# dobraczka/kiez

Hardware: AMD Instinct MI355X
Metric: source queries/sec (fit+kneighbors) + recall@k vs reference, 1/2/4/8 GPU (higher is better)
Workload: dtype f16

## Files before the change

kiez_amd/csrc/kz_knn_device.h:

```cpp
#pragma once
#include "kz_common.h"
#include "kz_plan.h"

typedef float f32x16 __attribute__((ext_vector_type(16)));
typedef float f32x4v __attribute__((ext_vector_type(4)));
__device__ __forceinline__ void kz_glds16(const float* gsrc, float* lds_wave_base) {
    __builtin_amdgcn_global_load_lds((const __attribute__((address_space(1))) void*)gsrc,
                                     (__attribute__((address_space(3))) void*)lds_wave_base, 16, 0, 0);
}
__device__ __forceinline__ void kz_glds16_s(const void* sbase_uniform, unsigned lane_byte_off, float* lds_wave_base) {
    const unsigned lds = (unsigned)(uintptr_t)(__attribute__((address_space(3))) void*)lds_wave_base;
    asm volatile("s_mov_b32 m0, %0\n\ts_nop 0\n\tglobal_load_lds_dwordx4 %1, %2"
                 :
                 : "s"(lds), "v"(lane_byte_off), "s"(sbase_uniform)
                 : "memory", "m0");
}
__device__ __forceinline__ void kz_glds4_s(const void* sbase_uniform, unsigned lane_byte_off, float* lds_wave_base) {
    const unsigned lds = (unsigned)(uintptr_t)(__attribute__((address_space(3))) void*)lds_wave_base;
    asm volatile("s_mov_b32 m0, %0\n\ts_nop 0\n\tglobal_load_lds_dword %1, %2"
                 :
                 : "s"(lds), "v"(lane_byte_off), "s"(sbase_uniform)
                 : "memory", "m0");
}
typedef float f32x4e __attribute__((ext_vector_type(4)));
typedef int i32x2e __attribute__((ext_vector_type(2)));
__device__ __forceinline__ float4 kz_nt_load4(const float4* p) {
    const f32x4v v = __builtin_nontemporal_load(reinterpret_cast<const f32x4v*>(p));
    return make_float4(v.x, v.y, v.z, v.w);
}


__host__ __device__ __forceinline__ int kz_list_region(int64_t list_row, const KzListLayout& L) {
    const int qt = (int)(list_row / KZ_TILE);
    int r = 0;
    while (r + 1 < L.n_regions && qt >= L.qt_end[r]) ++r;
    return r;
}
constexpr int KZ_LSTRIDE = 64;
__host__ __device__ __forceinline__ int64_t kz_list_wave_base(int64_t list_row, const KzListLayout& L, int KP, int piece) {
    const int r = kz_list_region(list_row, L);
    const int64_t row0 = r > 0 ? (int64_t)L.qt_end[r - 1] * KZ_TILE : 0;
    const int64_t wb = (list_row - row0) >> 5;
    return L.base[r] + ((wb * L.pieces[r] + piece) * (int64_t)KP) * KZ_LSTRIDE;
}

__host__ __device__ __forceinline__ int64_t kz_list_contig_off(int64_t list_row, const KzListLayout& L, int KP, int piece) {
    const int r = kz_list_region(list_row, L);
    const int64_t row0 = r > 0 ? (int64_t)L.qt_end[r - 1] * KZ_TILE : 0;
    return L.base[r] + ((list_row - row0) * L.pieces[r] + piece) * (int64_t)KP;
}

struct KnnCandParams {
    const float* qpack;
    const float* ypack;
    const float* ybias;
    const int4* work;
    int qt0;
    int n_ytiles;
    int n_qtiles;
    KzListLayout lay;
    int kg;
    float* out_key;
    int* out_idx;
    const float* theta;
    const float* qnbias;
    void* log_keys;
    void* log_meta;
    unsigned long long* log_cnt;
    long long log_cap;
    const float* qfloor;
};

constexpr int KZ_CAND_LDS_BASE = 16384 + 1024;
constexpr int KZ_LOG_CAP = 16;
constexpr int KZ_CAND_LDS = KZ_CAND_LDS_BASE + KZ_LOG_CAP * 256 * 8;

#ifndef KZ_SCAN_CHUNK
#define KZ_SCAN_CHUNK 16
#endif

template <int KP, int LSTRIDE, int CHUNK = KZ_SCAN_CHUNK>
__device__ __forceinline__ void kz_list_replace_min(float* lk, int* li, float v, int idx, float& tau, int& minpos) {
    lk[minpos * LSTRIDE] = v;
    li[minpos * LSTRIDE] = idx;
    float mn = INFINITY;
    int mp = 0;
#pragma unroll
    for (int c0 = 0; c0 < KP; c0 += CHUNK) {
        float kk[CHUNK];
#pragma unroll
        for (int e = 0; e < CHUNK; ++e) kk[e] = lk[(c0 + e) * LSTRIDE];
        __builtin_amdgcn_sched_barrier(0);
#pragma unroll
        for (int e = 0; e < CHUNK; ++e) {
            if (kk[e] < mn) {
                mn = kk[e];
                mp = c0 + e;
            }
        }
    }
    tau = mn;
    minpos = mp;
}


// ... 256 lines not shown
```

kiez_amd/csrc/kz_knn_epi3.h:

```cpp
#pragma once

typedef __attribute__((address_space(3))) float kz_lds_f32;
typedef __attribute__((address_space(3))) int kz_lds_i32;

template <int IN_LDS>
struct KzListRef;
template <>
struct KzListRef<1> {
    kz_lds_f32* k;
    int i_off;
    static constexpr int KSTRIDE = 128, ISTRIDE = 128;
    __device__ __forceinline__ kz_lds_f32* kp() const { return k; }
    __device__ __forceinline__ kz_lds_i32* ip() const { return (kz_lds_i32*)(k + i_off); }
};
template <>
struct KzListRef<0> {
    float* kb;
    int* ib;
    unsigned off;
    static constexpr int KSTRIDE = 1, ISTRIDE = 1;
    __device__ __forceinline__ float* kp() const { return kb + off; }
    __device__ __forceinline__ int* ip() const { return ib + off; }
};
template <>
struct KzListRef<2> {
    kz_lds_f32* k;
    int* ib;
    unsigned off_u, stride;
    static constexpr int KSTRIDE = 128, ISTRIDE = 1;
    __device__ __forceinline__ kz_lds_f32* kp() const { return k; }
    __device__ __forceinline__ int* ip() const {
        unsigned l;
        asm volatile("v_mbcnt_lo_u32_b32 %0, -1, 0\n\tv_mbcnt_hi_u32_b32 %0, -1, %0" : "=v"(l));
        return ib + off_u + (l & 31u) * stride;
    }
};

template <int IN_LDS>
struct KzCandState3 {
    KzListRef<IN_LDS> list;
    float tau;
    int head;
};

struct KzWavePool {
    __attribute__((address_space(3))) f32x4e* keys;
    __attribute__((address_space(3))) i32x2e* meta;
    int cnt;
    int tiles_done, next_merge;
};

struct KzDualRef {
    int qrow0;
};
constexpr int KZ_COL_FLAG = (int)0x80000000;

__device__ __forceinline__ void kz_flush_col3(const KzWavePool& pool, const KzDualRef& du) {
    const int lane = threadIdx.x & 63;
    int n_col = 0;
    for (int e0 = 0; e0 < pool.cnt; e0 += 64) {
        const int e = e0 + lane;
        const bool col = e < pool.cnt && pool.meta[e].x < 0;
        n_col += (int)__popcll(__builtin_amdgcn_ballot_w64(col));
    }
    if (n_col == 0) return;
    typedef __attribute__((address_space(4))) const volatile unsigned long long kz_karg_u64;
    const __attribute__((address_space(4))) char* ka = (const __attribute__((address_space(4))) char*)__builtin_amdgcn_kernarg_segment_ptr();
    f32x4e* log_keys = (f32x4e*)*(kz_karg_u64*)(ka + offsetof(KnnCandParams, log_keys));
    i32x2e* log_meta = (i32x2e*)*(kz_karg_u64*)(ka + offsetof(KnnCandParams, log_meta));
    unsigned long long* log_cnt = (unsigned long long*)*(kz_karg_u64*)(ka + offsetof(KnnCandParams, log_cnt));
    const long long log_cap = (long long)*(kz_karg_u64*)(ka + offsetof(KnnCandParams, log_cap));
    unsigned long long base = 0;
    if (lane == 0) base = __hip_atomic_fetch_add(log_cnt, (unsigned long long)n_col, __ATOMIC_RELAXED, __HIP_MEMORY_SCOPE_AGENT);
    base = ((unsigned long long)__builtin_amdgcn_readfirstlane((int)(base >> 32)) << 32) | (unsigned)__builtin_amdgcn_readfirstlane((int)base);
    for (int e0 = 0; e0 < pool.cnt; e0 += 64) {
        const int e = e0 + lane;
        i32x2e mt;
        mt.x = 0;
        if (e < pool.cnt) mt = pool.meta[e];
        const bool col = mt.x < 0;
        const unsigned long long mask = __builtin_amdgcn_ballot_w64(col);
        if (col) {
            const unsigned long long pos = base + __builtin_amdgcn_mbcnt_hi((unsigned)(mask >> 32), __builtin_amdgcn_mbcnt_lo((unsigned)mask, 0u));
            if ((long long)pos < log_cap) {
                i32x2e mo;
                mo.x = mt.x & 0x7fffffff;
                mo.y = du.qrow0 + (mt.x & 31);
                __builtin_nontemporal_store(pool.keys[e], log_keys + pos);
                __builtin_nontemporal_store(mo, log_meta + pos);
            }
        }
        base += __popcll(mask);
    }
}

template <int KP>
struct KzBlockMin3 {
    static constexpr int NB = KP >= 64 ? 8 : 4;
    static constexpr int BS = KP / NB;
    float bm[NB];
    __device__ __forceinline__ void init(const float v) {
#pragma unroll
        for (int i = 0; i < NB; ++i) bm[i] = v;
    }
};

template <int KP, int IN_LDS>
__device__ __forceinline__ void kz_list_insert3(const KzListRef<IN_LDS>& L, KzBlockMin3<KP>& bs, float v, int idx, float& tau) {
    constexpr int NB = KzBlockMin3<KP>::NB, BS = KzBlockMin3<KP>::BS, S = KzListRef<IN_LDS>::KSTRIDE, SI = KzListRef<IN_LDS>::ISTRIDE;
    float m = bs.bm[0];
    int b = 0;
#pragma unroll
    for (int i = 1; i < NB; ++i) {
        if (bs.bm[i] < m) {
            m = bs.bm[i];
            b = i;
        }
    }
    auto* blk = L.kp() + (b * BS) * S;
    float kk[BS];
#pragma unroll
    for (int jj = 0; jj < BS; ++jj) kk[jj] = blk[jj * S];
    int pos = BS - 1;
#pragma unroll
    for (int jj = BS - 2; jj >= 0; --jj) pos = (kk[jj] == m) ? jj : pos;
    blk[pos * S] = v;
    L.ip()[(b * BS + pos) * SI] = idx;
    float nm = INFINITY;
#pragma unroll
    for (int jj = 0; jj < BS; ++jj) nm = fminf(nm, (jj == pos) ? v : kk[jj]);
    float t = INFINITY;
#pragma unroll
    for (int i = 0; i < NB; ++i) {
        bs.bm[i] = (b == i) ? nm : bs.bm[i];
        t = fminf(t, bs.bm[i]);
    }
    tau = t;
}

template <int KP, int IN_LDS>
__device__ __forceinline__ void kz_insert_group3(const KzListRef<IN_LDS>& L, KzBlockMin3<KP>& bs,
                                                 __attribute__((address_space(3))) f32x4e* entry,
                                                 const __attribute__((address_space(3))) i32x2e* meta, const int half, float& tau) {
    auto row_of = [&]() {
        const int code = meta->x;
        return (code >> 4) * KZ_TILE + ((code >> 2) & 3) * 32 + (code & 3) * 8 + 4 * half;
    };
    {
        const f32x4e kv = *entry;
        const float m = fmaxf(fmaxf(kv.x, kv.y), fmaxf(kv.z, kv.w));
        if (!(m > tau)) return;
        const int slot = kv.x == m ? 0 : (kv.y == m ? 1 : (kv.z == m ? 2 : 3));
        reinterpret_cast<__attribute__((address_space(3))) float*>(entry)[slot] = -INFINITY;
// ... 223 lines not shown
```

kiez_amd/csrc/kz_knn_epi4.h:

```cpp
#pragma once
#include "kz_knn_epi3.h"

struct KzCandState4 {
    KzListRef<1> list;
    float tau[2];
    int head[2];
};

struct KzDualRef4 {
    int qrow0;
};
constexpr int KZ_COL_QH = 0x40000000;

__device__ __forceinline__ void kz_flush_col4(const KzWavePool& pool, const KzDualRef4& du) {
    const int lane = threadIdx.x & 63;
    int n_col = 0;
    for (int e0 = 0; e0 < pool.cnt; e0 += 64) {
        const int e = e0 + lane;
        const bool col = e < pool.cnt && pool.meta[e].x < 0;
        n_col += (int)__popcll(__builtin_amdgcn_ballot_w64(col));
    }
    if (n_col == 0) return;
    typedef __attribute__((address_space(4))) const volatile unsigned long long kz_karg_u64;
    const __attribute__((address_space(4))) char* ka = (const __attribute__((address_space(4))) char*)__builtin_amdgcn_kernarg_segment_ptr();
    f32x4e* log_keys = (f32x4e*)*(kz_karg_u64*)(ka + offsetof(KnnCandParams, log_keys));
    i32x2e* log_meta = (i32x2e*)*(kz_karg_u64*)(ka + offsetof(KnnCandParams, log_meta));
    unsigned long long* log_cnt = (unsigned long long*)*(kz_karg_u64*)(ka + offsetof(KnnCandParams, log_cnt));
    const long long log_cap = (long long)*(kz_karg_u64*)(ka + offsetof(KnnCandParams, log_cap));
    unsigned long long base = 0;
    if (lane == 0) base = __hip_atomic_fetch_add(log_cnt, (unsigned long long)n_col, __ATOMIC_RELAXED, __HIP_MEMORY_SCOPE_AGENT);
    base = ((unsigned long long)__builtin_amdgcn_readfirstlane((int)(base >> 32)) << 32) | (unsigned)__builtin_amdgcn_readfirstlane((int)base);
    for (int e0 = 0; e0 < pool.cnt; e0 += 64) {
        const int e = e0 + lane;
        i32x2e mt;
        mt.x = 0;
        if (e < pool.cnt) mt = pool.meta[e];
        const bool col = mt.x < 0;
        const unsigned long long mask = __builtin_amdgcn_ballot_w64(col);
        if (col) {
            const unsigned long long pos = base + __builtin_amdgcn_mbcnt_hi((unsigned)(mask >> 32), __builtin_amdgcn_mbcnt_lo((unsigned)mask, 0u));
            if ((long long)pos < log_cap) {
                i32x2e mo;
                mo.x = mt.x & 0x3fffffff;
                mo.y = du.qrow0 + ((mt.x & KZ_COL_QH) ? 32 : 0) + (mt.x & 31);
                __builtin_nontemporal_store(pool.keys[e], log_keys + pos);
                __builtin_nontemporal_store(mo, log_meta + pos);
            }
        }
        base += __popcll(mask);
    }
}

template <bool DUAL>
__device__ __forceinline__ void kz_merge_pool4(KzCandState4& st, KzWavePool& pool, const KzDualRef4& du) {
    constexpr int KP = 16;
    const int lane = threadIdx.x & 63;
    if constexpr (DUAL) kz_flush_col4(pool, du);
#pragma unroll 1
    for (int qh = 0; qh < 2; ++qh) {
        const int own = qh ? st.head[1] : st.head[0];
        const int other = __shfl_xor(own, 32, 64);
        float tau = qh ? st.tau[1] : st.tau[0];
        if (lane < 32) {
            KzListRef<1> L = st.list;
            L.k += 32 * qh;
            KzBlockMin3<KP> bs;
            constexpr int NB = KzBlockMin3<KP>::NB, BS = KzBlockMin3<KP>::BS, S = KzListRef<1>::KSTRIDE;
#pragma unroll
            for (int b = 0; b < NB; ++b) {
                float m = INFINITY;
#pragma unroll
                for (int jj = 0; jj < BS; ++jj) m = fminf(m, L.kp()[(b * BS + jj) * S]);
                bs.bm[b] = m;
            }
#pragma unroll 1
            for (int half = 0; half < 2; ++half) {
                int e = half ? other : own;
#pragma unroll 1
                while (e >= 0) {
                    auto* entry = pool.keys + e;
                    const auto* meta = pool.meta + e;
                    e = meta->y;
                    kz_insert_group3<KP, 1>(L, bs, entry, meta, half, tau);
                }
            }
        }
        tau = __shfl(tau, lane & 31, 64);
        if (qh) {
            st.tau[1] = tau;
            st.head[1] = -1;
        } else {
            st.tau[0] = tau;
            st.head[0] = -1;
        }
    }
    pool.cnt = 0;
}

#define KZ_EPI4_APPEND(blk, g4, gi, head, ev, mask)                                                                   \
    do {                                                                                                              \
        if (ev) {                                                                                                     \
            const int pos = pool.cnt + (int)__builtin_amdgcn_mbcnt_hi((unsigned)((mask) >> 32),                       \
                                                                      __builtin_amdgcn_mbcnt_lo((unsigned)(mask), 0u)); \
            f32x4e kv;                                                                                                \
            kv.x = (blk)[4 * (g4)];                                                                                   \
            kv.y = (blk)[4 * (g4) + 1];                                                                               \
            kv.z = (blk)[4 * (g4) + 2];                                                                               \
            kv.w = (blk)[4 * (g4) + 3];                                                                               \
            pool.keys[pos] = kv;                                                                                      \
            { i32x2e mv_; mv_.x = tile * 16 + (gi); mv_.y = (head); pool.meta[pos] = mv_; }                           \
// ... 156 lines not shown
```

kiez_amd/csrc/kz_knn_h16.h:

```cpp
#pragma once
#include <type_traits>

#include "kz_knn_epi3.h"

typedef _Float16 kz_f16x8 __attribute__((ext_vector_type(8)));

#ifndef KZ_H_DMA_LATE
#define KZ_H_DMA_LATE 1
#endif
template <int KP, int WPS, int NSR, bool DUAL = false, bool WIDE = false>
struct KzHCfg {
    static constexpr int TPW = WIDE ? WPS : 1;
    static constexpr bool LDS_LIST = KP <= 32;
    static constexpr bool LISTS_FIT = WPS <= 2 || KP == 16;
    static constexpr int LMODE = (LDS_LIST && LISTS_FIT) ? 1 : (((KP == 64 && WPS <= 2) || (KP == 32 && WPS == 3)) ? 2 : 0);
    static constexpr bool IN_LDS = LMODE == 1;
    static constexpr int RING = WIDE ? 8 : (WPS == 1 ? 8 : ((WPS == 3 || KP == 32 || NSR < 4) ? 4 : 8));
    static constexpr int PERIOD = RING / 2;
    static constexpr int CAP = WPS == 3 ? (KP <= 32 ? (DUAL ? 176 : 192) : 256) : (WPS == 2 && LMODE == 2 && RING == 8 ? (DUAL ? 140 : 156) : 256);
    static constexpr int RING_BYTES = RING * 4096;
    static constexpr int BIAS_OFF = RING_BYTES;
    static constexpr int SYNC_OFF = BIAS_OFF + 1024;
    static constexpr int THETA_OFF = SYNC_OFF + 256;
    static constexpr int POOLK_OFF = THETA_OFF + (DUAL ? 768 + 768 * TPW : 0);
// ... 32 lines not shown
#endif
    const int t_begin = wd.y, t_end = wd.z, s = wd.w;
    const int total = (t_end - t_begin) * NSR;
    const int wq = WIDE ? (wave & 3) : wave;
    const int wq_v = WIDE ? ((tid >> 6) & 3) : (tid >> 6);
    const int tb = WIDE ? (wave >> 2) : 0;
    const bool valid = !WIDE || wd.x + tb < p.n_qtiles;
    const int qt = WIDE ? (valid ? wd.x + tb : p.n_qtiles - 1) : wd.x;

    auto out_list_offset = [&]() { return kz_list_contig_off((int64_t)qt * KZ_TILE + 32 * wq_v + j, p.lay, KP, s); };
    KzCandState3<IN_LDS> st;
    if constexpr (IN_LDS == 1) {
        st.list.k = (kz_lds_f32*)(smem + Cfg::LIST_OFF + tb * Cfg::LIST_BLOCK) + 32 * wq_v + j;
        st.list.i_off = KP * 128;
    } else if constexpr (IN_LDS == 2) {
        st.list.k = (kz_lds_f32*)(smem + Cfg::LIST_OFF + tb * Cfg::LIST_BLOCK) + 32 * wq_v + j;
        st.list.ib = p.out_idx;
        {
            const int64_t row0 = (int64_t)qt * KZ_TILE + 32 * wq;
            const int64_t o0 = kz_list_contig_off(row0, p.lay, KP, s);
            st.list.off_u = (unsigned)o0;
            st.list.stride = (unsigned)(kz_list_contig_off(row0 + 1, p.lay, KP, s) - o0);
        }
    } else {
        st.list.kb = p.out_key;
        st.list.ib = p.out_idx;
        st.list.off = (unsigned)out_list_offset();
    }
    KzWavePool pool;
    pool.keys = (__attribute__((address_space(3))) f32x4e*)(smem + Cfg::POOLK_OFF) + wave * CAP;
    pool.meta = (__attribute__((address_space(3))) i32x2e*)(smem + Cfg::POOLM_OFF) + wave * CAP;
    const float fl = p.qfloor ? p.qfloor[(int64_t)(p.qt0 + qt) * KZ_TILE + 32 * wq_v + j] : -INFINITY;
    if (h == 0 && valid) {
#pragma unroll 4
        for (int e = 0; e < KP; ++e) {
            st.list.kp()[e * KzListRef<IN_LDS>::KSTRIDE] = fl;
            st.list.ip()[e * KzListRef<IN_LDS>::ISTRIDE] = -1;
        }
    }
    if (total <= 0) {
        if constexpr (IN_LDS != 0) {
            const int64_t listoff = out_list_offset();
            if (h == 0 && valid)
                for (int e = 0; e < KP; ++e) {
                    p.out_key[listoff + e] = -INFINITY;
                    if constexpr (IN_LDS == 1) p.out_idx[listoff + e] = -1;
                }
        }
        return;
    }
    st.tau = valid ? fl : INFINITY;
    KzBlockMin3<KP> bmin;
    bmin.init(fl);
    st.head = -1;
    pool.cnt = 0;
    pool.tiles_done = 0;
    pool.next_merge = 1;

    const char* dma_src = reinterpret_cast<const char*>(p.ypack) + ((int64_t)t_begin * NSR) * 4096;
    int dma_slot = 0;
    int dma_turn = 0;
    const int lane_off = (WIDE ? (tid & 255) : tid) * 16;
    auto dma_next = [&]() {
        float* dst = ybuf + dma_slot * 1024 + wq * 256;
        if (!WIDE || tb == dma_turn) kz_glds16_s(dma_src, (unsigned)lane_off, dst);
        if constexpr (WIDE) dma_turn = dma_turn + 1 == TPW ? 0 : dma_turn + 1;
        dma_src += 4096;
        dma_slot = (dma_slot + 1) & (R - 1);
    };
#pragma unroll
    for (int i = 0; i < R; ++i) dma_next();
    bbuf[(t_begin & 1) * 128 + (tid & 127)] = p.ybias[(int64_t)t_begin * KZ_TILE + (tid & 127)];
    KzDualRef du;
    if constexpr (DUAL) {
        if (tid < 64) tbuf[tid] = p.theta[(int64_t)t_begin * KZ_TILE + tid];
        du.qrow0 = (p.qt0 + qt) * KZ_TILE + 32 * wq;
        if (h == 0) tbuf[192 + 32 * (tid >> 6) + j] = valid ? p.qnbias[du.qrow0 + j] : INFINITY;
    }
    if (tid < 4) msync[tid] = 0;
    const float* qbase = p.qpack + ((int64_t)(p.qt0 + qt) * NSR) * 1024 + (h * KZ_TILE + 32 * wq_v + j) * 4;
    kz_f16x8 qf[NSR];
#pragma unroll
    for (int u = 0; u < NSR; ++u) qf[u] = *reinterpret_cast<const kz_f16x8*>(qbase + u * 1024);
    asm volatile("s_waitcnt vmcnt(0)" ::: "memory");
    __syncthreads();

    const float* fbase = ybuf + (h * KZ_TILE + j) * 4;
    kz_f16x8 f0[4], f1[4];
    int dma_due = 0;
    auto fetch_frags = [&](kz_f16x8 (&f)[4], const int gi) {
        const float* fb = fbase + (gi & (R - 1)) * 1024;
#pragma unroll
        for (int mt = 0; mt < 4; ++mt) f[mt] = *reinterpret_cast<const kz_f16x8*>(fb + 128 * mt);
    };
    if (CARRY) fetch_frags(f0, 0);
    int g = 0;
    int th_cur = 0;
    f32x16 acc[4];

    auto run_tile = [&](const int tile, auto start_parity) __attribute__((always_inline)) {
        constexpr int P0 = decltype(start_parity)::value;
        {
            int h_now = h;
            if constexpr (WPS == 3) {
                asm volatile("v_mbcnt_lo_u32_b32 %0, -1, 0\n\tv_mbcnt_hi_u32_b32 %0, -1, %0\n\tv_lshrrev_b32 %0, 5, %0" : "=v"(h_now));
            }
            const float* bp = bbuf + (tile & 1) * 128 + 4 * h_now;
#pragma unroll
            for (int mt = 0; mt < 4; ++mt) {
#pragma unroll
                for (int g4 = 0; g4 < 4; ++g4) {
                    const float4 v = *reinterpret_cast<const float4*>(bp + 32 * mt + 8 * g4);
                    acc[mt][4 * g4 + 0] = v.x;
                    acc[mt][4 * g4 + 1] = v.y;
                    acc[mt][4 * g4 + 2] = v.z;
                    acc[mt][4 * g4 + 3] = v.w;
                }
            }
        }
        __builtin_amdgcn_sched_barrier(0);
        {
            unsigned off4;
            asm volatile("v_lshrrev_b32 %0, 2, %1" : "=v"(off4) : "v"(lane_off));
            if (wave < 2)
                kz_glds4_s(p.ybias + (int64_t)min(tile + 1, p.n_ytiles - 1) * KZ_TILE, off4, bbuf + ((tile + 1) & 1) * 128 + wave * 64);
            else if (DUAL && wave == 2)
                kz_glds4_s(p.theta + ((int64_t)min(tile + 1, p.n_ytiles - 1) - 1) * KZ_TILE, off4, tbuf + (th_cur == 2 ? 0 : th_cur + 1) * 64);
        }
        constexpr bool carry_in = !ONE_SET && (CARRY || (P0 == 1 && (NSR & 1)));
        constexpr bool carry_out = !ONE_SET && (CARRY || (((P0 + NSR) & 1) != 0));
        if (!carry_in && !ONE_SET) {
            if (P0)
                fetch_frags(f1, g);
            else
                fetch_frags(f0, g);
        }
#pragma unroll
        for (int u = 0; u < NSR; ++u) {
            const bool odd = ((P0 + u) & 1) != 0;
            kz_f16x8 (&cur)[4] = (odd && !ONE_SET) ? f1 : f0;
            __builtin_amdgcn_sched_barrier(0);
            if (ONE_SET) {
                fetch_frags(f0, g);
            } else if (carry_out || u + 1 < NSR) {
                if (odd)
                    fetch_frags(f0, g + 1);
                else
                    fetch_frags(f1, g + 1);
            }
            __builtin_amdgcn_sched_barrier(0);
#pragma unroll
            for (int mt = 0; mt < 4; ++mt) acc[mt] = __builtin_amdgcn_mfma_f32_32x32x16_f16(cur[mt], qf[u], acc[mt], 0, 0, 0);
            if constexpr (LATE) {
                if (dma_due) {
#pragma unroll
                    for (int i = 0; i < P; ++i) dma_next();
                    dma_due = 0;
                }
            }
            if ((ONE_SET ? odd : !odd) && (P == 2 || ((g + LAG) & (P - 1)) == 0)) {
                asm volatile("s_waitcnt vmcnt(0) lgkmcnt(0)\n\ts_barrier" ::: "memory");
                if constexpr (LATE) {
                    dma_due = 1;
                } else {
                    {
#pragma unroll
                        for (int i = 0; i < P; ++i) dma_next();
// ... 58 lines not shown
```

kiez_amd/csrc/kz_knn_h64.h:

```cpp
#pragma once
#include <type_traits>

#include "kz_knn_epi4.h"
#include "kz_knn_h16.h"

template <int NSR, bool DUAL>
struct KzH64Cfg {
    static constexpr int KP = 16;
    static constexpr int RING = 8, PERIOD = 4;
    static constexpr int SLOT_FLOATS = 512;
    static constexpr int CAP = 288;
    static constexpr int RING_BYTES = RING * SLOT_FLOATS * 4;
    static constexpr int BIAS_OFF = RING_BYTES;
    static constexpr int SYNC_OFF = BIAS_OFF + 512;
    static constexpr int THETA_OFF = SYNC_OFF + 256;
    static constexpr int POOLK_OFF = THETA_OFF + (DUAL ? 768 + 1024 : 0);
    static constexpr int POOLM_OFF = POOLK_OFF + 4 * CAP * 16;
    static constexpr int LIST_OFF = POOLM_OFF + 4 * CAP * 8;
    static constexpr int LIST_BLOCK = KP * 128 * 8;
    static constexpr int LDS_BYTES = LIST_OFF + 2 * LIST_BLOCK;
    static_assert(LDS_BYTES <= 64 * 1280, "two workgroups per CU: 64 LDS granules of 1280 B each");
    static_assert(NSR >= PERIOD && NSR <= 13, "every half tile must contain a slice barrier; 13 stationary slices = 104 VGPRs");
};

template <int NSR, bool DUAL>
__global__ __launch_bounds__(256, 2) void kz_knn_cand_h64_kernel(KnnCandParams p) {
    using Cfg = KzH64Cfg<NSR, DUAL>;
    constexpr int R = Cfg::RING, P = Cfg::PERIOD, CAP = Cfg::CAP, KP = Cfg::KP;
    static_assert(R == 2 * P && (R & (R - 1)) == 0, "a power-of-two ring of two periods");
    extern __shared__ __attribute__((aligned(16))) char smem[];
    float* ybuf = reinterpret_cast<float*>(smem);
    float* bbuf = reinterpret_cast<float*>(smem + Cfg::BIAS_OFF);
    float* tbuf = reinterpret_cast<float*>(smem + Cfg::THETA_OFF);
    kz_lds_i32* msync = (kz_lds_i32*)(smem + Cfg::SYNC_OFF);
    const int tid = threadIdx.x;
    const int lane = tid & 63;
    const int wave = __builtin_amdgcn_readfirstlane(tid >> 6);
    const int j = lane & 31;
    const int h = lane >> 5;
    const int4 wd = p.work[blockIdx.x];
    const int t_begin = wd.y, t_end = wd.z, s = wd.w;
    const int tb = wave >> 1;
    const int r0 = 64 * (wave & 1);
    const int r0_v = 64 * ((tid >> 6) & 1);
    const bool valid = wd.x + tb < p.n_qtiles;
    const int qt = valid ? wd.x + tb : p.n_qtiles - 1;

    auto out_list_offset = [&](const int qh) { return kz_list_contig_off((int64_t)qt * KZ_TILE + r0_v + 32 * qh + j, p.lay, KP, s); };
    KzCandState4 st;
    st.list.k = (kz_lds_f32*)(smem + Cfg::LIST_OFF + tb * Cfg::LIST_BLOCK) + r0_v + j;
    st.list.i_off = KP * 128;
    KzWavePool pool;
    pool.keys = (__attribute__((address_space(3))) f32x4e*)(smem + Cfg::POOLK_OFF) + wave * CAP;
    pool.meta = (__attribute__((address_space(3))) i32x2e*)(smem + Cfg::POOLM_OFF) + wave * CAP;
    const int64_t frow = (int64_t)(p.qt0 + qt) * KZ_TILE + r0_v + j;
    const float fl0 = p.qfloor ? p.qfloor[frow] : -INFINITY, fl1 = p.qfloor ? p.qfloor[frow + 32] : -INFINITY;
    if (h == 0 && valid) {
#pragma unroll 4
        for (int e = 0; e < KP; ++e) {
            st.list.kp()[e * 128] = fl0;
            st.list.kp()[e * 128 + 32] = fl1;
            st.list.ip()[e * 128] = -1;
            st.list.ip()[e * 128 + 32] = -1;
        }
    }
    if (t_end <= t_begin) {
        if (h == 0 && valid) {
#pragma unroll 1
            for (int qh = 0; qh < 2; ++qh) {
                const int64_t listoff = out_list_offset(qh);
                for (int e = 0; e < KP; ++e) {
                    p.out_key[listoff + e] = -INFINITY;
                    p.out_idx[listoff + e] = -1;
                }
            }
        }
        return;
    }
    st.tau[0] = valid ? fl0 : INFINITY;
    st.tau[1] = valid ? fl1 : INFINITY;
    st.head[0] = st.head[1] = -1;
    pool.cnt = 0;
    pool.tiles_done = 0;
    pool.next_merge = 1;

    int d_tile = t_begin, d_hf = 0, d_u = tb, d_slot = tb;
    const char* ybase = reinterpret_cast<const char*>(p.ypack) + (wave & 1) * 2048;
    auto dma_next = [&]() {
        const char* src = ybase + ((int64_t)d_tile * NSR + d_u) * 4096 + d_hf * 1024;
        unsigned lane16;
        asm volatile("v_mbcnt_lo_u32_b32 %0, -1, 0\n\tv_mbcnt_hi_u32_b32 %0, -1, %0\n\tv_lshlrev_b32 %0, 4, %0" : "=v"(lane16));
        kz_glds16_s(src, lane16, ybuf + d_slot * Cfg::SLOT_FLOATS + (wave & 1) * 256);
        d_u += 2;
        if (d_u >= NSR) {
            d_u -= NSR;
            d_hf ^= 1;
            if (d_hf == 0) ++d_tile;
        }
        d_slot = (d_slot + 2) & (R - 1);
    };
#pragma unroll
    for (int i = 0; i < R / 2; ++i) dma_next();
    if (tid < 64) bbuf[tid] = p.ybias[(int64_t)t_begin * KZ_TILE + tid];
    KzDualRef4 du;
    du.qrow0 = (p.qt0 + qt) * KZ_TILE + r0;
    if constexpr (DUAL) {
        if (tid < 64) tbuf[tid] = p.theta[(int64_t)t_begin * KZ_TILE + tid];
        if (h == 0) {
            tbuf[192 + 64 * (tid >> 6) + j] = valid ? p.qnbias[du.qrow0 + j] : INFINITY;
            tbuf[192 + 64 * (tid >> 6) + 32 + j] = valid ? p.qnbias[du.qrow0 + 32 + j] : INFINITY;
        }
    }
    if (tid < 4) msync[tid] = 0;
    const float* qbase = p.qpack + ((int64_t)(p.qt0 + qt) * NSR) * 1024 + (h * KZ_TILE + r0_v + j) * 4;
    kz_f16x8 qf[2][NSR];
#pragma unroll
    for (int u = 0; u < NSR; ++u) {
        qf[0][u] = *reinterpret_cast<const kz_f16x8*>(qbase + u * 1024);
        qf[1][u] = *reinterpret_cast<const kz_f16x8*>(qbase + u * 1024 + 32 * 4);
    }
    asm volatile("s_waitcnt vmcnt(0)" ::: "memory");
    __syncthreads();

    const float* fbase = ybuf + (h * 64 + j) * 4;
    kz_f16x8 f0[2], f1[2];
    auto fetch_frags = [&](kz_f16x8 (&f)[2], const int gi) {
        const float* fb = fbase + (gi & (R - 1)) * Cfg::SLOT_FLOATS;
        f[0] = *reinterpret_cast<const kz_f16x8*>(fb);
        f[1] = *reinterpret_cast<const kz_f16x8*>(fb + 128);
    };
    fetch_frags(f0, 0);
    int g = 0;
    int seq = 0;
    int th_cur = 0;
    f32x16 acc[2][2];

    auto run_half = [&](const int tile, const int hf, auto start_parity) {
        constexpr int P0 = decltype(start_parity)::value;
        f32x16 binit[2];
        {
            const float* bp = bbuf + (seq & 1) * 64 + 4 * h;
#pragma unroll
            for (int rb = 0; rb < 2; ++rb) {
#pragma unroll
                for (int g4 = 0; g4 < 4; ++g4) {
                    const float4 v = *reinterpret_cast<const float4*>(bp + 32 * rb + 8 * g4);
                    binit[rb][4 * g4 + 0] = v.x;
                    binit[rb][4 * g4 + 1] = v.y;
                    binit[rb][4 * g4 + 2] = v.z;
                    binit[rb][4 * g4 + 3] = v.w;
                }
            }
        }
        __builtin_amdgcn_sched_barrier(0);
        {
            const int nt = hf ? min(tile + 1, p.n_ytiles - 1) : tile;
            unsigned lane4;
            asm volatile("v_mbcnt_lo_u32_b32 %0, -1, 0\n\tv_mbcnt_hi_u32_b32 %0, -1, %0\n\tv_lshlrev_b32 %0, 2, %0" : "=v"(lane4));
            if (wave == 0)
                kz_glds4_s(p.ybias + (int64_t)nt * KZ_TILE + (hf ? 0 : 64), lane4, bbuf + ((seq + 1) & 1) * 64);
            else if (DUAL && wave == 2)
                kz_glds4_s(p.theta + (int64_t)nt * KZ_TILE, lane4, tbuf + (th_cur == 2 ? 0 : th_cur + 1) * 64);
        }
#pragma unroll
        for (int u = 0; u < NSR; ++u) {
            const bool odd = ((P0 + u) & 1) != 0;
            kz_f16x8 (&cur)[2] = odd ? f1 : f0;
            __builtin_amdgcn_sched_barrier(0);
            if (odd)
                fetch_frags(f0, g + 1);
            else
                fetch_frags(f1, g + 1);
            __builtin_amdgcn_sched_barrier(0);
            if (u == 0) {
#pragma unroll
                for (int rb = 0; rb < 2; ++rb) {
                    acc[rb][1] = __builtin_amdgcn_mfma_f32_32x32x16_f16(cur[rb], qf[1][0], binit[rb], 0, 0, 0);
                    acc[rb][0] = __builtin_amdgcn_mfma_f32_32x32x16_f16(cur[rb], qf[0][0], binit[rb], 0, 0, 0);
                }
            } else {
#pragma unroll
                for (int rb = 0; rb < 2; ++rb) {
                    acc[rb][0] = __builtin_amdgcn_mfma_f32_32x32x16_f16(cur[rb], qf[0][u], acc[rb][0], 0, 0, 0);
                    acc[rb][1] = __builtin_amdgcn_mfma_f32_32x32x16_f16(cur[rb], qf[1][u], acc[rb][1], 0, 0, 0);
                }
            }
            if (((g + 2) & (P - 1)) == 0) {
                asm volatile("s_waitcnt vmcnt(0) lgkmcnt(0)\n\ts_barrier" ::: "memory");
#pragma unroll
                for (int i = 0; i < P / 2; ++i) dma_next();
            }
            ++g;
        }
        __builtin_amdgcn_sched_barrier(0);
        float cthr0 = INFINITY, cthr1 = INFINITY;
        if constexpr (DUAL) {
            const float th = tbuf[th_cur * 64];
            cthr0 = tbuf[192 + 64 * (tid >> 6) + j] + th;
            cthr1 = tbuf[192 + 64 * (tid >> 6) + 32 + j] + th;
            th_cur = th_cur == 2 ? 0 : th_cur + 1;
        }
        kz_half_epilogue4<CAP, DUAL>(acc, st, pool, tile, hf, hf == 1 && tile == t_end - 1, msync, du, cthr0, cthr1);
        ++seq;
    };

    int tile = t_begin;
    for (;;) {
        run_half(tile, 0, std::integral_constant<int, 0>{});
        run_half(tile, 1, std::integral_constant<int, (NSR & 1)>{});
        if (++tile >= t_end) break;
    }
    int lane_now;
    asm volatile("v_mbcnt_lo_u32_b32 %0, -1, 0\n\tv_mbcnt_hi_u32_b32 %0, -1, %0" : "=v"(lane_now));
    if (lane_now < 32 && valid) {
#pragma unroll 1
        for (int qh = 0; qh < 2; ++qh) {
            const int64_t listoff = out_list_offset(qh);
#pragma unroll 4
            for (int e = 0; e < KP; ++e) {
                p.out_key[listoff + e] = st.list.kp()[e * 128 + 32 * qh];
                p.out_idx[listoff + e] = st.list.ip()[e * 128 + 32 * qh];
            }
        }
    }
}
```

kiez_amd/csrc/kz_knn_hx16.h:

```cpp
#pragma once
#include "kz_knn_epi3.h"
#include "kz_knn_h16.h"

template <int KP, bool DUAL = false>
struct KzHxCfg {
    static constexpr int LMODE = KP <= 32 ? 1 : (KP == 64 ? 2 : 0);
    static constexpr int RING = 8, PERIOD = 4;
    static constexpr int CAP = 256;
    static constexpr int RING_BYTES = RING * 4096;
    static constexpr int BIAS_OFF = RING_BYTES;
    static constexpr int SYNC_OFF = BIAS_OFF + 1024;
    static constexpr int THETA_OFF = SYNC_OFF + 256;
    static constexpr int POOLK_OFF = THETA_OFF + (DUAL ? 768 + 768 : 0);
    static constexpr int POOLM_OFF = POOLK_OFF + 2 * CAP * 16;
    static constexpr int LIST_OFF = POOLM_OFF + 2 * CAP * 8;
    static constexpr int LIST_BLOCK = LMODE == 1 ? KP * 128 * 8 : (LMODE == 2 ? KP * 128 * 4 : 0);
    static constexpr int XBUF_OFF = LIST_OFF + LIST_BLOCK;
    static constexpr int XBUF_WAVE = 16 * 64 * 16;
    static constexpr int LDS_BYTES = XBUF_OFF + 4 * XBUF_WAVE;
    static_assert(LDS_BYTES <= 160 * 1024, "workgroup exceeds the CU's LDS");
};

template <int KP, int NS, bool DUAL = false>
__global__ __launch_bounds__(256, 1) void kz_knn_cand_hx_kernel(KnnCandParams p) {
// ... 25 lines not shown
            half = (b >> 3) & 1;
        } else {
            item = full + ((b - 2 * full) >> 1);
            half = b & 1;
        }
    }
    const int4 wd = p.work[item];
    const int qt = wd.x, t_begin = wd.y, t_end = wd.z, s = wd.w;
    const int total = (t_end - t_begin) * NS;
    const int qr = 64 * half + 32 * grp_v + j;

    auto out_list_offset = [&]() { return kz_list_contig_off((int64_t)qt * KZ_TILE + qr, p.lay, KP, s); };
    KzCandState3<IN_LDS> st;
    if constexpr (IN_LDS == 1) {
        st.list.k = (kz_lds_f32*)(smem + Cfg::LIST_OFF) + 32 * grp_v + j;
        st.list.i_off = KP * 128;
    } else if constexpr (IN_LDS == 2) {
        st.list.k = (kz_lds_f32*)(smem + Cfg::LIST_OFF) + 32 * grp_v + j;
        st.list.ib = p.out_idx;
        {
            const int64_t row0 = (int64_t)qt * KZ_TILE + 64 * half + 32 * grp;
            const int64_t o0 = kz_list_contig_off(row0, p.lay, KP, s);
            st.list.off_u = (unsigned)o0;
            st.list.stride = (unsigned)(kz_list_contig_off(row0 + 1, p.lay, KP, s) - o0);
        }
    } else {
        st.list.kb = p.out_key;
        st.list.ib = p.out_idx;
        st.list.off = (unsigned)out_list_offset();
    }
    KzWavePool pool;
    pool.keys = (__attribute__((address_space(3))) f32x4e*)(smem + Cfg::POOLK_OFF) + grp * CAP;
    pool.meta = (__attribute__((address_space(3))) i32x2e*)(smem + Cfg::POOLM_OFF) + grp * CAP;
    const float fl = p.qfloor ? p.qfloor[(int64_t)(p.qt0 + qt) * KZ_TILE + qr] : -INFINITY;
    if (h == 0 && kh == 0) {
#pragma unroll 4
        for (int e = 0; e < KP; ++e) {
            st.list.kp()[e * KzListRef<IN_LDS>::KSTRIDE] = fl;
            st.list.ip()[e * KzListRef<IN_LDS>::ISTRIDE] = -1;
        }
    }
    if (total <= 0) {
        if constexpr (IN_LDS != 0) {
            const int64_t listoff = out_list_offset();
            if (h == 0 && kh == 0)
                for (int e = 0; e < KP; ++e) {
                    p.out_key[listoff + e] = -INFINITY;
                    if constexpr (IN_LDS == 1) p.out_idx[listoff + e] = -1;
                }
        }
        return;
    }
    st.tau = fl;
    KzBlockMin3<KP> bmin;
    bmin.init(fl);
    st.head = -1;
    pool.cnt = 0;
    pool.tiles_done = 0;
    pool.next_merge = 1;

    const char* dma_src = reinterpret_cast<const char*>(p.ypack) + ((int64_t)t_begin * NS) * 4096;
    int dma_slot = 0;
    const int lane_off = tid * 16;
    auto dma_next = [&]() {
        float* dst = ybuf + dma_slot * 1024 + wave * 256;
        kz_glds16_s(dma_src, (unsigned)lane_off, dst);
        dma_src += 4096;
        dma_slot = (dma_slot + 1) & (R - 1);
    };
#pragma unroll
    for (int i = 0; i < R; ++i) dma_next();
    bbuf[(t_begin & 1) * 128 + (tid & 127)] = p.ybias[(int64_t)t_begin * KZ_TILE + (tid & 127)];
    KzDualRef du;
    if constexpr (DUAL) {
        if (tid < 64) tbuf[tid] = p.theta[(int64_t)t_begin * KZ_TILE + tid];
        du.qrow0 = (p.qt0 + qt) * KZ_TILE + 64 * half + 32 * grp;
        if (h == 0 && kh == 0) tbuf[192 + 32 * grp_v + j] = p.qnbias[du.qrow0 + j];
    }
    if (tid < 4) msync[tid] = 0;
    const float* qbase = p.qpack + ((int64_t)(p.qt0 + qt) * NS + kh) * 1024 + (h * KZ_TILE + qr) * 4;
    kz_f16x8 qf[NSH];
#pragma unroll
    for (int u = 0; u < NSH; ++u) qf[u] = *reinterpret_cast<const kz_f16x8*>(qbase + u * 2048);
    asm volatile("s_waitcnt vmcnt(0)" ::: "memory");
    __syncthreads();

    const float* fbase = ybuf + (h * KZ_TILE + j) * 4;
    kz_f16x8 f0[4], f1[4];
    int dma_due = 0;
    auto fetch_frags = [&](kz_f16x8 (&f)[4], const int gi) {
        const float* fb = fbase + (gi & (R - 1)) * 1024;
#pragma unroll
        for (int mt = 0; mt < 4; ++mt) f[mt] = *reinterpret_cast<const kz_f16x8*>(fb + 128 * mt);
    };
    fetch_frags(f0, kh);
    int g = 0;
    int th_cur = 0;
    f32x16 acc[4];
    typedef __attribute__((address_space(3))) f32x4e kz_lds_f32x4;

    auto run_tile = [&](const int tile) __attribute__((always_inline)) {
        if (kh == 0) {
            int h_now;
            asm volatile("v_mbcnt_lo_u32_b32 %0, -1, 0\n\tv_mbcnt_hi_u32_b32 %0, -1, %0\n\tv_lshrrev_b32 %0, 5, %0" : "=v"(h_now));
            const float* bp = bbuf + (tile & 1) * 128 + 4 * h_now;
#pragma unroll
            for (int mt = 0; mt < 4; ++mt) {
#pragma unroll
                for (int g4 = 0; g4 < 4; ++g4) {
                    const float4 v = *reinterpret_cast<const float4*>(bp + 32 * mt + 8 * g4);
                    acc[mt][4 * g4 + 0] = v.x;
                    acc[mt][4 * g4 + 1] = v.y;
                    acc[mt][4 * g4 + 2] = v.z;
                    acc[mt][4 * g4 + 3] = v.w;
                }
            }
        } else {
#pragma unroll
            for (int mt = 0; mt < 4; ++mt) {
#pragma unroll
                for (int i = 0; i < 16; ++i) acc[mt][i] = 0.0f;
            }
        }
        __builtin_amdgcn_sched_barrier(0);
        {
            unsigned off4;
            asm volatile("v_lshrrev_b32 %0, 2, %1" : "=v"(off4) : "v"(lane_off));
            if (wave < 2)
                kz_glds4_s(p.ybias + (int64_t)min(tile + 1, p.n_ytiles - 1) * KZ_TILE, off4, bbuf + ((tile + 1) & 1) * 128 + wave * 64);
            else if (DUAL && wave == 2)
                kz_glds4_s(p.theta + ((int64_t)min(tile + 1, p.n_ytiles - 1) - 1) * KZ_TILE, off4, tbuf + (th_cur == 2 ? 0 : th_cur + 1) * 64);
        }
#pragma unroll
        for (int u = 0; u < NS; ++u) {
            const bool mine = (u & 1) == kh;
            const bool set1 = ((u >> 1) & 1) != 0;
            kz_f16x8 (&cur)[4] = set1 ? f1 : f0;
            __builtin_amdgcn_sched_barrier(0);
            if (mine) {
                if (set1)
                    fetch_frags(f0, g + 2);
                else
                    fetch_frags(f1, g + 2);
            }
            __builtin_amdgcn_sched_barrier(0);
            if (mine) {
#pragma unroll
                for (int mt = 0; mt < 4; ++mt) acc[mt] = __builtin_amdgcn_mfma_f32_32x32x16_f16(cur[mt], qf[u >> 1], acc[mt], 0, 0, 0);
            }
            if (dma_due) {
#pragma unroll
                for (int i = 0; i < P; ++i) dma_next();
                dma_due = 0;
            }
            if ((u & 3) == 1) {
                asm volatile("s_waitcnt vmcnt(0) lgkmcnt(0)\n\ts_barrier" ::: "memory");
                dma_due = 1;
            }
            ++g;
        }
        __builtin_amdgcn_sched_barrier(0);
        int lane_x;
        asm volatile("v_mbcnt_lo_u32_b32 %0, -1, 0\n\tv_mbcnt_hi_u32_b32 %0, -1, %0" : "=v"(lane_x));
        kz_lds_f32x4* const xb = (kz_lds_f32x4*)(smem + Cfg::XBUF_OFF) + ((tile & 1) * 2 + grp) * (Cfg::XBUF_WAVE / 16) + lane_x;
        if (kh != 0) {
#pragma unroll
            for (int mt = 0; mt < 4; ++mt) {
// ... 50 lines not shown
```

Baseline: 2.483 million.

## Precompute DMA slice offsets at compile time and unroll tile loop by parity

The h64 kernel's runtime DMA cursor state (tile, half, slice, slot, with carry logic) is replaced by a constexpr offset function indexed by the compile-time slice position. The tile loop is unrolled twice when NSR is odd so the barrier phase stays a compile-time constant. This is meant to remove scalar and vector bookkeeping from the inner MFMA loop. Separately, the inline-asm vmcnt(0) waits become a builtin s_waitcnt so the compiler can see them, and the log pointers get an explicit global address space so flat accesses become global ones.

```diff
diff --git a/kiez_amd/csrc/kz_knn_device.h b/kiez_amd/csrc/kz_knn_device.h
--- a/kiez_amd/csrc/kz_knn_device.h
+++ b/kiez_amd/csrc/kz_knn_device.h
@@ -21,6 +21,11 @@
                  :
                  : "s"(lds), "v"(lane_byte_off), "s"(sbase_uniform)
                  : "memory", "m0");
+}
+__device__ __forceinline__ void kz_wait_vm0_seen() {
+    asm volatile("" ::: "memory");
+    __builtin_amdgcn_s_waitcnt(0x0f70);
+    asm volatile("" ::: "memory");
 }
 typedef float f32x4e __attribute__((ext_vector_type(4)));
 typedef int i32x2e __attribute__((ext_vector_type(2)));
diff --git a/kiez_amd/csrc/kz_knn_epi3.h b/kiez_amd/csrc/kz_knn_epi3.h
--- a/kiez_amd/csrc/kz_knn_epi3.h
+++ b/kiez_amd/csrc/kz_knn_epi3.h
@@ -54,6 +54,9 @@
     int qrow0;
 };
 constexpr int KZ_COL_FLAG = (int)0x80000000;
+typedef __attribute__((address_space(1))) f32x4e kz_glb_f32x4;
+typedef __attribute__((address_space(1))) i32x2e kz_glb_i32x2;
+typedef __attribute__((address_space(1))) unsigned long long kz_glb_u64;
 
 __device__ __forceinline__ void kz_flush_col3(const KzWavePool& pool, const KzDualRef& du) {
     const int lane = threadIdx.x & 63;
@@ -66,9 +69,9 @@
     if (n_col == 0) return;
     typedef __attribute__((address_space(4))) const volatile unsigned long long kz_karg_u64;
     const __attribute__((address_space(4))) char* ka = (const __attribute__((address_space(4))) char*)__builtin_amdgcn_kernarg_segment_ptr();
-    f32x4e* log_keys = (f32x4e*)*(kz_karg_u64*)(ka + offsetof(KnnCandParams, log_keys));
-    i32x2e* log_meta = (i32x2e*)*(kz_karg_u64*)(ka + offsetof(KnnCandParams, log_meta));
-    unsigned long long* log_cnt = (unsigned long long*)*(kz_karg_u64*)(ka + offsetof(KnnCandParams, log_cnt));
+    kz_glb_f32x4* log_keys = (kz_glb_f32x4*)*(kz_karg_u64*)(ka + offsetof(KnnCandParams, log_keys));
+    kz_glb_i32x2* log_meta = (kz_glb_i32x2*)*(kz_karg_u64*)(ka + offsetof(KnnCandParams, log_meta));
+    kz_glb_u64* log_cnt = (kz_glb_u64*)*(kz_karg_u64*)(ka + offsetof(KnnCandParams, log_cnt));
     const long long log_cap = (long long)*(kz_karg_u64*)(ka + offsetof(KnnCandParams, log_cap));
     unsigned long long base = 0;
     if (lane == 0) base = __hip_atomic_fetch_add(log_cnt, (unsigned long long)n_col, __ATOMIC_RELAXED, __HIP_MEMORY_SCOPE_AGENT);
diff --git a/kiez_amd/csrc/kz_knn_epi4.h b/kiez_amd/csrc/kz_knn_epi4.h
--- a/kiez_amd/csrc/kz_knn_epi4.h
+++ b/kiez_amd/csrc/kz_knn_epi4.h
@@ -23,9 +23,9 @@
     if (n_col == 0) return;
     typedef __attribute__((address_space(4))) const volatile unsigned long long kz_karg_u64;
     const __attribute__((address_space(4))) char* ka = (const __attribute__((address_space(4))) char*)__builtin_amdgcn_kernarg_segment_ptr();
-    f32x4e* log_keys = (f32x4e*)*(kz_karg_u64*)(ka + offsetof(KnnCandParams, log_keys));
-    i32x2e* log_meta = (i32x2e*)*(kz_karg_u64*)(ka + offsetof(KnnCandParams, log_meta));
-    unsigned long long* log_cnt = (unsigned long long*)*(kz_karg_u64*)(ka + offsetof(KnnCandParams, log_cnt));
+    kz_glb_f32x4* log_keys = (kz_glb_f32x4*)*(kz_karg_u64*)(ka + offsetof(KnnCandParams, log_keys));
+    kz_glb_i32x2* log_meta = (kz_glb_i32x2*)*(kz_karg_u64*)(ka + offsetof(KnnCandParams, log_meta));
+    kz_glb_u64* log_cnt = (kz_glb_u64*)*(kz_karg_u64*)(ka + offsetof(KnnCandParams, log_cnt));
     const long long log_cap = (long long)*(kz_karg_u64*)(ka + offsetof(KnnCandParams, log_cap));
     unsigned long long base = 0;
     if (lane == 0) base = __hip_atomic_fetch_add(log_cnt, (unsigned long long)n_col, __ATOMIC_RELAXED, __HIP_MEMORY_SCOPE_AGENT);
diff --git a/kiez_amd/csrc/kz_knn_h16.h b/kiez_amd/csrc/kz_knn_h16.h
--- a/kiez_amd/csrc/kz_knn_h16.h
+++ b/kiez_amd/csrc/kz_knn_h16.h
@@ -138,7 +138,7 @@
     kz_f16x8 qf[NSR];
 #pragma unroll
     for (int u = 0; u < NSR; ++u) qf[u] = *reinterpret_cast<const kz_f16x8*>(qbase + u * 1024);
-    asm volatile("s_waitcnt vmcnt(0)" ::: "memory");
+    kz_wait_vm0_seen();
     __syncthreads();
 
     const float* fbase = ybuf + (h * KZ_TILE + j) * 4;
diff --git a/kiez_amd/csrc/kz_knn_h64.h b/kiez_amd/csrc/kz_knn_h64.h
--- a/kiez_amd/csrc/kz_knn_h64.h
+++ b/kiez_amd/csrc/kz_knn_h64.h
@@ -22,6 +22,11 @@
     static_assert(LDS_BYTES <= 64 * 1280, "two workgroups per CU: 64 LDS granules of 1280 B each");
     static_assert(NSR >= PERIOD && NSR <= 13, "every half tile must contain a slice barrier; 13 stationary slices = 104 VGPRs");
 };
+
+template <int NSR>
+__host__ __device__ constexpr unsigned kz_h64_half_slice_off(const int L) {
+    return (unsigned)((L / (2 * NSR)) * NSR + (L % (2 * NSR)) % NSR) * 4096u + (unsigned)((L % (2 * NSR)) / NSR) * 1024u;
+}
 
 template <int NSR, bool DUAL>
 __global__ __launch_bounds__(256, 2) void kz_knn_cand_h64_kernel(KnnCandParams p) {
@@ -84,23 +89,17 @@
     pool.tiles_done = 0;
     pool.next_merge = 1;
 
-    int d_tile = t_begin, d_hf = 0, d_u = tb, d_slot = tb;
-    const char* ybase = reinterpret_cast<const char*>(p.ypack) + (wave & 1) * 2048;
-    auto dma_next = [&]() {
-        const char* src = ybase + ((int64_t)d_tile * NSR + d_u) * 4096 + d_hf * 1024;
+    const char* tile_src = reinterpret_cast<const char*>(p.ypack) + (wave & 1) * 2048 + ((int64_t)t_begin * NSR) * 4096;
+    float* const ring_wave = ybuf + tb * Cfg::SLOT_FLOATS + (wave & 1) * 256;
+    int ring_hi = 0;
+    auto dma_at = [&](const int L0, const int slot0) __attribute__((always_inline)) {
+        const unsigned off = tb ? kz_h64_half_slice_off<NSR>(L0 + 1) : kz_h64_half_slice_off<NSR>(L0);
         unsigned lane16;
         asm volatile("v_mbcnt_lo_u32_b32 %0, -1, 0\n\tv_mbcnt_hi_u32_b32 %0, -1, %0\n\tv_lshlrev_b32 %0, 4, %0" : "=v"(lane16));
-        kz_glds16_s(src, lane16, ybuf + d_slot * Cfg::SLOT_FLOATS + (wave & 1) * 256);
-        d_u += 2;
-        if (d_u >= NSR) {
-            d_u -= NSR;
-            d_hf ^= 1;
-            if (d_hf == 0) ++d_tile;
-        }
-        d_slot = (d_slot + 2) & (R - 1);
+        kz_glds16_s(tile_src + off, lane16, ring_wave + slot0 * Cfg::SLOT_FLOATS);
     };
 #pragma unroll
-    for (int i = 0; i < R / 2; ++i) dma_next();
+    for (int i = 0; i < R / 2; ++i) dma_at(2 * i, 2 * i);
     if (tid < 64) bbuf[tid] = p.ybias[(int64_t)t_begin * KZ_TILE + tid];
     KzDualRef4 du;
     du.qrow0 = (p.qt0 + qt) * KZ_TILE + r0;
@@ -119,7 +118,7 @@
         qf[0][u] = *reinterpret_cast<const kz_f16x8*>(qbase + u * 1024);
         qf[1][u] = *reinterpret_cast<const kz_f16x8*>(qbase + u * 1024 + 32 * 4);
     }
-    asm volatile("s_waitcnt vmcnt(0)" ::: "memory");
+    kz_wait_vm0_seen();
     __syncthreads();
 
     const float* fbase = ybuf + (h * 64 + j) * 4;
@@ -135,8 +134,9 @@
     int th_cur = 0;
     f32x16 acc[2][2];
 
-    auto run_half = [&](const int tile, const int hf, auto start_parity) {
-        constexpr int P0 = decltype(start_parity)::value;
+    auto run_half = [&](const int tile, auto half, auto start_phase) __attribute__((always_inline)) {
+        constexpr int HF = decltype(half)::value, Q0 = decltype(start_phase)::value, P0 = Q0 & 1;
+        const int hf = HF;
         f32x16 binit[2];
         {
             const float* bp = bbuf + (seq & 1) * 64 + 4 * h;
@@ -185,10 +185,11 @@
                     acc[rb][1] = __builtin_amdgcn_mfma_f32_32x32x16_f16(cur[rb], qf[1][u], acc[rb][1], 0, 0, 0);
                 }
             }
-            if (((g + 2) & (P - 1)) == 0) {
+            if (((Q0 + u + 2) & (P - 1)) == 0) {
                 asm volatile("s_waitcnt vmcnt(0) lgkmcnt(0)\n\ts_barrier" ::: "memory");
-#pragma unroll
-                for (int i = 0; i < P / 2; ++i) dma_next();
+                dma_at(HF * NSR + u + 6, ring_hi);
+                dma_at(HF * NSR + u + 8, ring_hi + 2);
+                ring_hi ^= 4;
             }
             ++g;
         }
@@ -204,11 +205,20 @@
         ++seq;
     };
 
+    using H0 = std::integral_constant<int, 0>;
+    using H1 = std::integral_constant<int, 1>;
     int tile = t_begin;
     for (;;) {
-        run_half(tile, 0, std::integral_constant<int, 0>{});
-        run_half(tile, 1, std::integral_constant<int, (NSR & 1)>{});
+        run_half(tile, H0{}, std::integral_constant<int, 0>{});
+        run_half(tile, H1{}, std::integral_constant<int, NSR % P>{});
+        tile_src += NSR * 4096;
         if (++tile >= t_end) break;
+        if constexpr ((NSR & 1) != 0) {
+            run_half(tile, H0{}, std::integral_constant<int, 2>{});
+            run_half(tile, H1{}, std::integral_constant<int, (2 + NSR) % P>{});
+            tile_src += NSR * 4096;
+            if (++tile >= t_end) break;
+        }
     }
     int lane_now;
     asm volatile("v_mbcnt_lo_u32_b32 %0, -1, 0\n\tv_mbcnt_hi_u32_b32 %0, -1, %0" : "=v"(lane_now));
diff --git a/kiez_amd/csrc/kz_knn_hx16.h b/kiez_amd/csrc/kz_knn_hx16.h
--- a/kiez_amd/csrc/kz_knn_hx16.h
+++ b/kiez_amd/csrc/kz_knn_hx16.h
@@ -131,7 +131,7 @@
     kz_f16x8 qf[NSH];
 #pragma unroll
     for (int u = 0; u < NSH; ++u) qf[u] = *reinterpret_cast<const kz_f16x8*>(qbase + u * 2048);
-    asm volatile("s_waitcnt vmcnt(0)" ::: "memory");
+    kz_wait_vm0_seen();
     __syncthreads();
 
     const float* fbase = ybuf + (h * KZ_TILE + j) * 4;
```

After: 2.642 million, median of 6. +6.4%, better.
